# retab-dev/k-LLMs

Measured on NVIDIA H100. Metric: consensus records/sec at n=16 (1M x 32-field); achieved HBM GB/s vs peak, higher is better.
Workload: dtype i32 codes / f64 values

## Files before the change

### k_llms_b200/csrc/kc_jsongpu.cu

```cuda
#include <cuda_runtime.h>

#include <algorithm>
#include <atomic>
#include <chrono>
#include <cstdio>
#include <cstdlib>
#include <cstring>
#include <mutex>
#include <string>
#include <thread>
#include <vector>

#include <cub/device/device_scan.cuh>
#include <nvtx3/nvToolsExt.h>

#include "../../include/kllms_b200.h"
#include "kc_internal.h"
#include "kc_jsongpu.cuh"

namespace {

using kc::js::Chunk;
using kc::js::Tok;

struct DBuf {
    void *p = nullptr;
    size_t cap = 0;
    int reserve(size_t need) {
        if (p && need <= cap) return KC_OK;
        if (p) cudaFree(p);
        p = nullptr;
        cap = 0;
        need += need / 8 + 256;
        if (cudaMalloc(&p, need) != cudaSuccess) {
            cudaGetLastError();
            return kc_fail(KC_ENOMEM, "kc_consolidate_json_packed: cudaMalloc(%zu) failed", need);
        }
        cap = need;
        return KC_OK;
    }
    template <typename T>
    T *as() const { return static_cast<T *>(p); }
};

struct PBuf {
    void *p = nullptr;
    size_t cap = 0;
    int reserve(size_t need) {
        if (p && need <= cap) return KC_OK;
        if (p) cudaFreeHost(p);
        p = nullptr;
        cap = 0;
        need += need / 8 + 256;
        if (cudaHostAlloc(&p, need, cudaHostAllocDefault) != cudaSuccess) {
            cudaGetLastError();
            return kc_fail(KC_ENOMEM, "kc_consolidate_json_packed: cudaHostAlloc(%zu) failed", need);
        }
        cap = need;
        return KC_OK;
    }
    template <typename T>
    T *as() const { return static_cast<T *>(p); }
};

struct Worker {
    int device = -1;
    cudaStream_t stream = nullptr;
    cudaEvent_t ev[7] = {};
    DBuf text, off, fcount, slot, status, vbase, xbase, counters, toks, fdesc, piece_c, piece_l, vcells, xcells, win, vmeta, xvalue, xmeta,
        len_c, len_l, out_c, out_l, scan_tmp, mcount, scount, ccount, mchars, mstr_off, mgrp_off, midx, mavg, nest, gpos;
    PBuf h_small;
    PBuf h_scan;
    bool busy = false;
    int init(int dev) {
        if (device == dev) return KC_OK;
        KC_CUDA_I(cudaStreamCreateWithFlags(&stream, cudaStreamNonBlocking));
        for (auto &e : ev) KC_CUDA_I(cudaEventCreate(&e));
        device = dev;
        return KC_OK;
    }
};

std::mutex g_pool_mu;
std::vector<Worker *> g_workers;

Worker *acquire_worker(int device) {
    std::lock_guard<std::mutex> lock(g_pool_mu);
    for (Worker *w : g_workers)
        if (!w->busy && w->device == device) {
            w->busy = true;
            return w;
        }
    Worker *w = new Worker;
    w->busy = true;
    g_workers.push_back(w);
    return w;
}
void release_worker(Worker *w) {
    std::lock_guard<std::mutex> lock(g_pool_mu);
    w->busy = false;
}

struct PinnedBlob {
    char *p = nullptr;
    size_t cap = 0;
};
std::vector<PinnedBlob> g_blob_pool;

PinnedBlob acquire_blob(size_t need) {
    {
        std::lock_guard<std::mutex> lock(g_pool_mu);
        int best = -1;
        for (int i = 0; i < (int)g_blob_pool.size(); ++i)
            if (g_blob_pool[i].cap >= need && (best < 0 || g_blob_pool[i].cap < g_blob_pool[best].cap)) best = i;
        if (best >= 0) {
            PinnedBlob b = g_blob_pool[best];
            g_blob_pool.erase(g_blob_pool.begin() + best);
            return b;
        }
    }
    PinnedBlob b;
    void *p = nullptr;
    if (cudaHostAlloc(&p, need, cudaHostAllocDefault) != cudaSuccess) {
        cudaGetLastError();
        return b;
    }
    b.p = (char *)p;
    b.cap = need;
    return b;
}
void release_blob(PinnedBlob b) {
    if (!b.p) return;
    std::lock_guard<std::mutex> lock(g_pool_mu);
    size_t n_small = 0, n_large = 0;
    for (auto &x : g_blob_pool) (x.cap <= ((size_t)4 << 20) ? n_small : n_large)++;
    if (b.cap <= ((size_t)4 << 20) && n_small < 64) {
        g_blob_pool.push_back(b);
        return;
    }
    if (n_large >= 4 || b.cap <= ((size_t)4 << 20)) {
        int smallest = -1;
        for (int i = 0; i < (int)g_blob_pool.size(); ++i)
            if (g_blob_pool[i].cap > ((size_t)4 << 20) && (smallest < 0 || g_blob_pool[i].cap < g_blob_pool[smallest].cap)) smallest = i;
        if (smallest < 0 || g_blob_pool[smallest].cap >= b.cap) {
            cudaFreeHost(b.p);
            return;
        }
        cudaFreeHost(g_blob_pool[smallest].p);
        g_blob_pool.erase(g_blob_pool.begin() + smallest);
    }
    g_blob_pool.push_back(b);
}

int team_size(int n) {
    int t = 2;
    while (t < n && t < 32) t *= 2;
    return t;
}

}

struct kc_json_result {
    int64_t R = 0;
    PinnedBlob blob;
    std::atomic<int64_t> used{0};
    std::vector<int64_t> c_off, c_len, l_off, l_len;
    std::vector<uint8_t> status, why;
    std::string heap;
    kc_json_stats stats{};
};

namespace {

struct ChunkStage {
    float h2d = 0, plan = 0, kernels = 0, emit = 0, d2h = 0;
};

int run_chunk(Worker &w, const char *h_text, const int64_t *h_off, int64_t r0, int64_t r1, int32_t n, double rel_eps, double abs_eps,
              int sm_count, kc_json_result &res, ChunkStage &st) {
    const int64_t Rc = r1 - r0;
    const int64_t b0 = h_off[r0 * n], b1 = h_off[r1 * n];
    const size_t bytes = (size_t)(b1 - b0);
    if (bytes >= ((size_t)1 << 32)) return kc_fail(KC_EINVAL, "kc_consolidate_json_packed: chunk of %zu bytes", bytes);
    cudaStream_t s = w.stream;
    int rc;
#define R_(call)          \
    do {                  \
        rc = (call);      \
        if (rc) return rc; \
    } while (0)
    R_(w.text.reserve(bytes + 16));
    R_(w.off.reserve((size_t)(Rc * n + 1) * 8));
    R_(w.fcount.reserve((size_t)(Rc + 1) * 4));
    R_(w.slot.reserve((size_t)(Rc + 1) * 4));
    R_(w.status.reserve((size_t)Rc));
    R_(w.nest.reserve((size_t)Rc));
    R_(w.vbase.reserve((size_t)Rc * 4));
    R_(w.xbase.reserve((size_t)Rc * 4));
    R_(w.counters.reserve(32));
    R_(w.mcount.reserve((size_t)(Rc + 1) * 4));
    R_(w.scount.reserve((size_t)(Rc + 1) * 4));
    R_(w.ccount.reserve((size_t)(Rc + 1) * 4));
    R_(w.len_c.reserve((size_t)(Rc + 1) * 8));
    R_(w.len_l.reserve((size_t)(Rc + 1) * 8));
    R_(w.h_small.reserve(64));
    R_(w.h_scan.reserve((size_t)(Rc + 1) * 16 + (size_t)Rc));
    size_t tmp_bytes = 0, tmp_bytes32 = 0;
    cub::DeviceScan::ExclusiveSum(nullptr, tmp_bytes, (const int64_t *)nullptr, (int64_t *)nullptr, (int)(Rc + 1), s);
    cub::DeviceScan::ExclusiveSum(nullptr, tmp_bytes32, (const uint32_t *)nullptr, (uint32_t *)nullptr, (int)(Rc + 1), s);
    R_(w.scan_tmp.reserve(std::max(tmp_bytes, tmp_bytes32) + 256));

    Chunk ch{};
    ch.text = w.text.as<uint8_t>();
    ch.off = w.off.as<int64_t>();
    ch.R = (int32_t)Rc;
    ch.n = n;
    ch.fcount = w.fcount.as<uint32_t>();
    ch.slot = w.slot.as<uint32_t>();
    ch.status = w.status.as<uint8_t>();
    ch.nest = w.nest.as<uint8_t>();
    ch.vbase = w.vbase.as<uint32_t>();
    ch.xbase = w.xbase.as<uint32_t>();
    ch.counters = w.counters.as<unsigned long long>();
    ch.mcount = w.mcount.as<uint32_t>();
    ch.scount = w.scount.as<uint32_t>();
    ch.ccount = w.ccount.as<uint32_t>();
    ch.len_c = w.len_c.as<int64_t>();
    ch.len_l = w.len_l.as<int64_t>();

    nvtxRangePushA("kc_json: H2D texts");
    KC_CUDA_I(cudaEventRecord(w.ev[0], s));
    KC_CUDA_I(cudaMemcpyAsync(w.text.p, h_text + b0, bytes, cudaMemcpyHostToDevice, s));
    KC_CUDA_I(cudaMemcpyAsync(w.off.p, h_off + r0 * n, (size_t)(Rc * n + 1) * 8, cudaMemcpyHostToDevice, s));
    KC_CUDA_I(cudaEventRecord(w.ev[1], s));
    nvtxRangePop();
    nvtxRangePushA("kc_json: plan (A0 count, A1 scan/type/encode)");

    const int team = team_size(n);
    const int tpw = 32 / team;
    auto grid_for = [&](int64_t threads_needed) {
        const int64_t blocks = (threads_needed + 127) / 128;
        return (int)std::max<int64_t>(1, std::min<int64_t>(blocks, (int64_t)sm_count * 16));
    };
    KC_CUDA_I(cudaMemsetAsync(ch.fcount + Rc, 0, 4, s));
    kc::js::count_kernel<<<grid_for(Rc), 128, 0, s>>>(ch);
    KC_CUDA_I(cudaGetLastError());
    size_t tb = w.scan_tmp.cap;
    KC_CUDA_I(cub::DeviceScan::ExclusiveSum(w.scan_tmp.p, tb, (const uint32_t *)ch.fcount, ch.slot, (int)(Rc + 1), s));
    uint32_t *h_total = w.h_small.as<uint32_t>();
    KC_CUDA_I(cudaMemcpyAsync(h_total, ch.slot + Rc, 4, cudaMemcpyDeviceToHost, s));
    KC_CUDA_I(cudaStreamSynchronize(s));
    const size_t T = *h_total;
    const size_t Tn = T * (size_t)n;
    R_(w.toks.reserve(std::max<size_t>(Tn, 1) * sizeof(Tok)));
    R_(w.fdesc.reserve(std::max<size_t>(T, 1) * 4));
    R_(w.gpos.reserve(std::max<size_t>(T, 1) * 4));
    R_(w.piece_c.reserve(std::max<size_t>(T, 1) * 4));
    R_(w.piece_l.reserve(std::max<size_t>(T, 1) * 4));
    R_(w.vcells.reserve(std::max<size_t>(Tn, 16)));
    R_(w.xcells.reserve(std::max<size_t>(Tn, 2) * 8));
    R_(w.win.reserve(std::max<size_t>(T, 1) * 4));
    R_(w.vmeta.reserve(std::max<size_t>(T, 1) * 4));
    R_(w.xvalue.reserve(std::max<size_t>(T, 1) * 8));
    R_(w.xmeta.reserve(std::max<size_t>(T, 1) * 4));
    ch.toks = w.toks.as<Tok>();
    ch.fdesc = w.fdesc.as<uint32_t>();
    ch.gpos = w.gpos.as<uint32_t>();
    ch.piece_c = w.piece_c.as<uint32_t>();
    ch.piece_l = w.piece_l.as<uint32_t>();
    ch.vcells = w.vcells.as<int8_t>();
    ch.xcells = w.xcells.as<double>();
    ch.vmeta = w.vmeta.as<uint32_t>();
    ch.xvalue = w.xvalue.as<double>();
    ch.xmeta = w.xmeta.as<uint32_t>();
    KC_CUDA_I(cudaMemsetAsync(w.counters.p, 0, 24, s));
    KC_CUDA_I(cudaMemsetAsync(w.mcount.p, 0, (size_t)(Rc + 1) * 4, s));
    KC_CUDA_I(cudaMemsetAsync(w.scount.p, 0, (size_t)(Rc + 1) * 4, s));
    KC_CUDA_I(cudaMemsetAsync(w.ccount.p, 0, (size_t)(Rc + 1) * 4, s));
    KC_CUDA_I(cudaMemsetAsync(w.vcells.p, 0xFF, std::max<size_t>(Tn, 16), s));
    KC_CUDA_I(cudaMemsetAsync(w.xcells.p, 0, std::max<size_t>(Tn, 2) * 8, s));
    int64_t gv = 0, gx = 0, gm = 0;
    if (T) {
        const int64_t rounds = (Rc + tpw - 1) / tpw;
        kc::js::plan_kernel<<<grid_for(rounds * 32), 128, 0, s>>>(ch, team);
        KC_CUDA_I(cudaGetLastError());
        unsigned long long *h_cnt = w.h_small.as<unsigned long long>() + 1;
        KC_CUDA_I(cudaMemcpyAsync(h_cnt, w.counters.p, 24, cudaMemcpyDeviceToHost, s));
        KC_CUDA_I(cudaStreamSynchronize(s));
        gv = (int64_t)h_cnt[0];
        gx = (int64_t)h_cnt[1];
        gm = (int64_t)h_cnt[2];
    }
    if (gm) {
        R_(w.mchars.reserve(bytes + 16));
        R_(w.mstr_off.reserve((Tn + 2) * 4));
        R_(w.mgrp_off.reserve((T + 2) * 4));
        R_(w.midx.reserve((T + 1) * 4));
        R_(w.mavg.reserve((T + 1) * 8));
        ch.mchars = w.mchars.as<uint8_t>();
        ch.mstr_off = w.mstr_off.as<int32_t>();
        ch.mgrp_off = w.mgrp_off.as<int32_t>();
        ch.midx = w.midx.as<int32_t>();
        ch.mavg = w.mavg.as<double>();
        for (uint32_t *cnt : {ch.mcount, ch.scount, ch.ccount}) {
            tb = w.scan_tmp.cap;
            KC_CUDA_I(cub::DeviceScan::ExclusiveSum(w.scan_tmp.p, tb, (const uint32_t *)cnt, cnt, (int)(Rc + 1), s));
        }
        const int64_t rounds = (Rc + tpw - 1) / tpw;
        kc::js::medoid_kernel<<<grid_for(rounds * 32), 128, 0, s>>>(ch, team);
        KC_CUDA_I(cudaGetLastError());
    }
    KC_CUDA_I(cudaEventRecord(w.ev[2], s));
    nvtxRangePop();
    nvtxRangePushA("kc_json: K1 vote + K2 numeric + K4 medoid");
    if (gv) R_(kc_vote_i8(ch.vcells, gv, n, nullptr, 1, w.win.as<int32_t>(), w.vmeta.as<uint32_t>(), s));
    if (gx) R_(kc_numeric_f64(ch.xcells, gx, n, rel_eps, abs_eps, w.xvalue.as<double>(), w.xmeta.as<uint32_t>(), s));
    if (gm) R_(kc_medoid_str(ch.mchars, ch.mstr_off, ch.mgrp_off, gm, std::max(2, n), w.midx.as<int32_t>(), w.mavg.as<double>(), s));
    KC_CUDA_I(cudaEventRecord(w.ev[3], s));
    nvtxRangePop();
    nvtxRangePushA("kc_json: emit (C0 lengths, C1 write)");
    KC_CUDA_I(cudaMemsetAsync(ch.len_c + Rc, 0, 8, s));
    KC_CUDA_I(cudaMemsetAsync(ch.len_l + Rc, 0, 8, s));
    {
        const int64_t rounds = (Rc + tpw - 1) / tpw;
        kc::js::len_kernel<<<grid_for(rounds * 32), 128, 0, s>>>(ch, team);
        KC_CUDA_I(cudaGetLastError());
    }
    tb = w.scan_tmp.cap;
    KC_CUDA_I(cub::DeviceScan::ExclusiveSum(w.scan_tmp.p, tb, (const int64_t *)ch.len_c, ch.len_c, (int)(Rc + 1), s));
    tb = w.scan_tmp.cap;
    KC_CUDA_I(cub::DeviceScan::ExclusiveSum(w.scan_tmp.p, tb, (const int64_t *)ch.len_l, ch.len_l, (int)(Rc + 1), s));
    int64_t *h_scan_c = w.h_scan.as<int64_t>(), *h_scan_l = h_scan_c + (Rc + 1);
    uint8_t *h_status = (uint8_t *)(h_scan_l + (Rc + 1));
    KC_CUDA_I(cudaMemcpyAsync(h_scan_c, ch.len_c, (size_t)(Rc + 1) * 8, cudaMemcpyDeviceToHost, s));
    KC_CUDA_I(cudaMemcpyAsync(h_scan_l, ch.len_l, (size_t)(Rc + 1) * 8, cudaMemcpyDeviceToHost, s));
    KC_CUDA_I(cudaMemcpyAsync(h_status, ch.status, (size_t)Rc, cudaMemcpyDeviceToHost, s));
    KC_CUDA_I(cudaStreamSynchronize(s));
    const int64_t out_c_bytes = h_scan_c[Rc], out_l_bytes = h_scan_l[Rc];
    R_(w.out_c.reserve((size_t)std::max<int64_t>(out_c_bytes, 1)));
    R_(w.out_l.reserve((size_t)std::max<int64_t>(out_l_bytes, 1)));
    ch.out_c = w.out_c.as<uint8_t>();
    ch.out_l = w.out_l.as<uint8_t>();
    if (out_c_bytes) {
        const int64_t rounds = (Rc + tpw - 1) / tpw;
        kc::js::write_kernel<<<grid_for(rounds * 32), 128, 0, s>>>(ch, team);
        KC_CUDA_I(cudaGetLastError());
    }
    KC_CUDA_I(cudaEventRecord(w.ev[4], s));
    nvtxRangePop();
    nvtxRangePushA("kc_json: D2H texts");
    const int64_t need = out_c_bytes + out_l_bytes;
    const int64_t pos = res.used.fetch_add(need);
    if (pos + need > (int64_t)res.blob.cap) {
        res.used.fetch_sub(need);
        for (int64_t r = r0; r < r1; ++r) {
            res.status[(size_t)r] = 1;
            res.why[(size_t)r] = (uint8_t)kc::js::D_TOO_LONG;
        }
        return KC_OK;
    }
    if (out_c_bytes) KC_CUDA_I(cudaMemcpyAsync(res.blob.p + pos, ch.out_c, (size_t)out_c_bytes, cudaMemcpyDeviceToHost, s));
    if (out_l_bytes) KC_CUDA_I(cudaMemcpyAsync(res.blob.p + pos + out_c_bytes, ch.out_l, (size_t)out_l_bytes, cudaMemcpyDeviceToHost, s));
    KC_CUDA_I(cudaEventRecord(w.ev[5], s));
    KC_CUDA_I(cudaStreamSynchronize(s));
    nvtxRangePop();
    for (int64_t i = 0; i < Rc; ++i) {
        const int64_t r = r0 + i;
        res.status[(size_t)r] = h_status[i] ? 1 : 0;
        res.why[(size_t)r] = h_status[i];
        res.c_off[(size_t)r] = pos + h_scan_c[i];
        res.c_len[(size_t)r] = h_scan_c[i + 1] - h_scan_c[i];
        res.l_off[(size_t)r] = pos + out_c_bytes + h_scan_l[i];
        res.l_len[(size_t)r] = h_scan_l[i + 1] - h_scan_l[i];
    }
    float ms = 0;
    cudaEventElapsedTime(&ms, w.ev[0], w.ev[1]); st.h2d += ms;
    cudaEventElapsedTime(&ms, w.ev[1], w.ev[2]); st.plan += ms;
    cudaEventElapsedTime(&ms, w.ev[2], w.ev[3]); st.kernels += ms;
    cudaEventElapsedTime(&ms, w.ev[3], w.ev[4]); st.emit += ms;
    cudaEventElapsedTime(&ms, w.ev[4], w.ev[5]); st.d2h += ms;
#undef R_
    return KC_OK;
}

}

extern "C" {

int kc_consolidate_json_packed(const char *h_text, const int64_t *h_off, int64_t n_records, int32_t n, double rel_eps, double abs_eps,
                               int device, int32_t threads, uint32_t flags, kc_json_result **out) {
    if (!out) return kc_fail(KC_EINVAL, "kc_consolidate_json_packed: NULL out");
    *out = nullptr;
    if (n < 2 || n > KC_MAX_CANDIDATES) return kc_fail(KC_EINVAL, "kc_consolidate_json_packed: n=%d outside [2,%d]", n, KC_MAX_CANDIDATES);
    if (n_records < 0 || (n_records && (!h_text || !h_off))) return kc_fail(KC_EINVAL, "kc_consolidate_json_packed: bad arguments");
    if (!(rel_eps >= 0.0) || !(abs_eps >= 0.0)) return kc_fail(KC_EINVAL, "kc_consolidate_json_packed: rel_eps/abs_eps must be >= 0");
    const auto t_start = std::chrono::steady_clock::now();
    int prev = 0;
    KC_CUDA_I(cudaGetDevice(&prev));
    KC_CUDA_I(cudaSetDevice(device));
    int sm_count = 0, cc_major = 0;
    KC_CUDA_I(cudaDeviceGetAttribute(&sm_count, cudaDevAttrMultiProcessorCount, device));
    KC_CUDA_I(cudaDeviceGetAttribute(&cc_major, cudaDevAttrComputeCapabilityMajor, device));
    if (cc_major != 9) {
        cudaSetDevice(prev);
        return kc_fail(KC_ENODEV, "device %d has compute capability %d.x; this library is sm_90a only", device, cc_major);
    }
    kc_json_result *res = new (std::nothrow) kc_json_result;
    if (!res) return kc_fail(KC_ENOMEM, "kc_consolidate_json_packed: out of memory");
    const int64_t R = n_records;
    res->R = R;
    res->c_off.assign((size_t)R, 0);
    res->c_len.assign((size_t)R, 0);
    res->l_off.assign((size_t)R, 0);
    res->l_len.assign((size_t)R, 0);
    res->status.assign((size_t)R, 1);
    res->why.assign((size_t)R, 0);
    const int64_t total_bytes = R ? h_off[R * n] - h_off[0] : 0;
    res->blob = acquire_blob((size_t)(total_bytes / n * 3 + (1 << 20)));
    if (!res->blob.p) {
        delete res;
        cudaSetDevice(prev);
        return kc_fail(KC_ENOMEM, "kc_consolidate_json_packed: cannot allocate the pinned output blob");
    }
    size_t chunk_bytes = (size_t)64 << 20;
    if (const char *e = getenv("KC_JSON_CHUNK_MB")) chunk_bytes = (size_t)std::min(1024, std::max(1, atoi(e))) << 20;
    std::vector<int64_t> cuts{0};
    {
        int64_t r = 0;
        while (r < R) {
            const int64_t start = h_off[r * n];
            int64_t lo = r + 1, hi = R;
            while (lo < hi) {
                const int64_t mid = lo + (hi - lo + 1) / 2;
                if ((size_t)(h_off[mid * n] - start) <= chunk_bytes) lo = mid;
                else hi = mid - 1;
            }
            r = lo;
            cuts.push_back(r);
        }
    }
    const int n_chunks = (int)cuts.size() - 1;
    int n_workers = 3;
    if (const char *e = getenv("KC_JSON_STREAMS")) n_workers = std::max(1, std::min(8, atoi(e)));
    n_workers = std::max(1, std::min(n_workers, n_chunks));
    std::vector<Worker *> workers;
    for (int i = 0; i < n_workers; ++i) workers.push_back(acquire_worker(device));
    std::vector<int> rcs((size_t)n_workers, KC_OK);
    std::vector<std::string> errs((size_t)n_workers);
    std::vector<ChunkStage> stages((size_t)n_workers);
    std::atomic<int> next{0};
    auto body = [&](int wi) {
        cudaSetDevice(device);
        Worker &w = *workers[(size_t)wi];
        int rc = w.init(device);
        while (!rc) {
            const int k = next.fetch_add(1);
            if (k >= n_chunks) break;
            rc = run_chunk(w, h_text, h_off, cuts[(size_t)k], cuts[(size_t)k + 1], n, rel_eps, abs_eps, sm_count, *res, stages[(size_t)wi]);
        }
        if (rc) {
            cudaStreamSynchronize(w.stream);
            errs[(size_t)wi] = kc_last_error();
        }
        rcs[(size_t)wi] = rc;
    };
    if (n_workers == 1) {
        body(0);
    } else {
        std::vector<std::thread> pool;
        for (int i = 0; i < n_workers; ++i) pool.emplace_back(body, i);
        for (auto &t : pool) t.join();
    }
    for (Worker *w : workers) release_worker(w);
    int rc = KC_OK;
    for (int i = 0; i < n_workers && !rc; ++i)
        if (rcs[(size_t)i]) rc = kc_fail(rcs[(size_t)i], "%s", errs[(size_t)i].c_str());
    const auto t_gpu = std::chrono::steady_clock::now();
    int64_t n_declined = 0, n_host = 0;
    if (!rc) {
        std::vector<int64_t> idx;
        for (int64_t r = 0; r < R; ++r)
            if (res->status[(size_t)r]) idx.push_back(r);
        n_declined = (int64_t)idx.size();
        if (!idx.empty() && !(flags & KC_JSON_DEVICE_ONLY)) {
            const int64_t D = (int64_t)idx.size();
            std::vector<const char *> texts((size_t)(D * n));
            std::vector<int64_t> lens((size_t)(D * n));
            for (int64_t i = 0; i < D; ++i)
                for (int32_t c = 0; c < n; ++c) {
                    const int64_t k = idx[(size_t)i] * n + c;
                    texts[(size_t)(i * n + c)] = h_text + h_off[k];
                    lens[(size_t)(i * n + c)] = h_off[k + 1] - h_off[k];
                }
            std::vector<char *> oc((size_t)D, nullptr), ol((size_t)D, nullptr);
            std::vector<uint8_t> hs((size_t)D, 1);
            rc = kc_consolidate_json(texts.data(), lens.data(), D, n, rel_eps, abs_eps, device, threads, oc.data(), ol.data(), hs.data());
            if (!rc) {
                int64_t pos = res->used.load(), extra = 0;
                for (int64_t i = 0; i < D; ++i)
                    if (hs[(size_t)i] == 0) extra += (int64_t)(strlen(oc[(size_t)i]) + strlen(ol[(size_t)i]));
                char *base = res->blob.p;
                if (pos + extra > (int64_t)res->blob.cap) {
                    res->heap.resize((size_t)(pos + extra));
                    memcpy(&res->heap[0], res->blob.p, (size_t)pos);
                    release_blob(res->blob);
                    res->blob = PinnedBlob{};
                    base = &res->heap[0];
                }
                for (int64_t i = 0; i < D; ++i) {
                    if (hs[(size_t)i] != 0) continue;
                    const int64_t r = idx[(size_t)i];
                    const size_t lc = strlen(oc[(size_t)i]), ll = strlen(ol[(size_t)i]);
                    memcpy(base + pos, oc[(size_t)i], lc);
                    memcpy(base + pos + lc, ol[(size_t)i], ll);
                    res->c_off[(size_t)r] = pos;
                    res->l_off[(size_t)r] = pos + (int64_t)lc;
                    res->c_len[(size_t)r] = (int64_t)lc;
                    res->l_len[(size_t)r] = (int64_t)ll;
                    res->status[(size_t)r] = 2;
                    pos += (int64_t)(lc + ll);
                    ++n_host;
                }
                res->used.store(pos);
            }
            kc_free_strings(oc.data(), D);
            kc_free_strings(ol.data(), D);
        }
    }
    cudaSetDevice(prev);
    if (rc) {
        release_blob(res->blob);
        delete res;
        return rc;
    }
    const auto t_end = std::chrono::steady_clock::now();
    auto ms = [](auto a, auto b) { return std::chrono::duration<double, std::milli>(b - a).count(); };
    kc_json_stats &s = res->stats;
    s.n_records = R;
    s.n_device = R - n_declined;
    s.n_host = n_host;
    s.n_python = n_declined - n_host;
    s.input_bytes = total_bytes;
    s.output_bytes = res->used.load();
    s.chunks = n_chunks;
    s.streams = n_workers;
    for (auto &g : stages) {
        s.h2d_ms += g.h2d;
        s.plan_ms += g.plan;
        s.kernel_ms += g.kernels;
        s.emit_ms += g.emit;
        s.d2h_ms += g.d2h;
    }
    s.device_path_wall_ms = ms(t_start, t_gpu);
    s.host_path_wall_ms = ms(t_gpu, t_end);
    s.wall_ms = ms(t_start, t_end);
    *out = res;
    return KC_OK;
}

int kc_json_result_view(kc_json_result *res, const char **text, const int64_t **content_off, const int64_t **content_len,
                        const int64_t **likelihoods_off, const int64_t **likelihoods_len, const uint8_t **status, const uint8_t **why,
                        kc_json_stats *stats) {
    if (!res) return kc_fail(KC_EINVAL, "kc_json_result_view: NULL result");
    if (text) *text = res->blob.p ? res->blob.p : res->heap.data();
    if (content_off) *content_off = res->c_off.data();
    if (content_len) *content_len = res->c_len.data();
    if (likelihoods_off) *likelihoods_off = res->l_off.data();
    if (likelihoods_len) *likelihoods_len = res->l_len.data();
    if (status) *status = res->status.data();
    if (why) *why = res->why.data();
    if (stats) *stats = res->stats;
    return KC_OK;
}

void kc_json_result_free(kc_json_result *res) {
    if (!res) return;
    release_blob(res->blob);
    delete res;
}


struct kc_debug_jsongpu {
    std::vector<int64_t> off;
    std::vector<uint8_t> text;
    int32_t n = 0;
    int64_t R = 0;
    std::vector<uint32_t> fcount, slot, fdesc, gpos, vbase, xbase, piece_c, piece_l;
    std::vector<uint8_t> status, nest;
    std::vector<Tok> toks;
    unsigned long long counters[3] = {0, 0, 0};
    std::vector<uint32_t> mcount, scount, ccount;
    std::vector<uint8_t> mchars;
    std::vector<int32_t> mstr_off, mgrp_off;
    std::vector<int8_t> vcells;
    std::vector<double> xcells;
    std::vector<int64_t> len_c, len_l;
    std::vector<uint8_t> out_c, out_l;
    Chunk ch{};
};

int kc_debug_jsongpu_plan(const char *h_text, const int64_t *h_off, int64_t n_records, int32_t n, kc_debug_jsongpu **out) {
    if (!h_text || !h_off || !out || n < 2 || n > KC_MAX_CANDIDATES || n_records < 0) return KC_EINVAL;
    kc_debug_jsongpu *h = new kc_debug_jsongpu;
    const int64_t R = n_records;
    h->R = R;
    h->n = n;
    h->off.assign(h_off, h_off + R * n + 1);
    h->text.assign((const uint8_t *)h_text + h_off[0], (const uint8_t *)h_text + h_off[R * n]);
    h->fcount.assign((size_t)R + 1, 0);
    h->slot.assign((size_t)R + 1, 0);
    h->status.assign((size_t)R, 0);
    h->nest.assign((size_t)R, 0);
    h->vbase.assign((size_t)R, 0);
    h->xbase.assign((size_t)R, 0);
    h->len_c.assign((size_t)R + 1, 0);
    h->len_l.assign((size_t)R + 1, 0);
    h->mcount.assign((size_t)R + 1, 0);
    h->scount.assign((size_t)R + 1, 0);
    h->ccount.assign((size_t)R + 1, 0);
    Chunk &ch = h->ch;
    ch.text = h->text.data();
    ch.off = h->off.data();
    ch.R = (int32_t)R;
    ch.n = n;
    ch.fcount = h->fcount.data();
    ch.slot = h->slot.data();
    ch.status = h->status.data();
    ch.nest = h->nest.data();
    ch.vbase = h->vbase.data();
    ch.xbase = h->xbase.data();
    ch.counters = h->counters;
    ch.mcount = h->mcount.data();
    ch.scount = h->scount.data();
    ch.ccount = h->ccount.data();
    ch.len_c = h->len_c.data();
    ch.len_l = h->len_l.data();
    for (int32_t r = 0; r < R; ++r) kc::js::count_record(ch, r);
    for (int64_t r = 0; r < R; ++r) h->slot[(size_t)r + 1] = h->slot[(size_t)r] + h->fcount[(size_t)r];
    const size_t T = h->slot[(size_t)R];
    h->toks.assign(std::max<size_t>(T * n, 1), Tok{});
    h->fdesc.assign(std::max<size_t>(T, 1), 0);
    h->gpos.assign(std::max<size_t>(T, 1), 0);
    h->piece_c.assign(std::max<size_t>(T, 1), 0);
    h->piece_l.assign(std::max<size_t>(T, 1), 0);
    h->vcells.assign(std::max<size_t>(T * n, 16), (int8_t)-1);
    h->xcells.assign(std::max<size_t>(T * n, 2), 0.0);
    ch.toks = h->toks.data();
    ch.fdesc = h->fdesc.data();
    ch.gpos = h->gpos.data();
    ch.piece_c = h->piece_c.data();
    ch.piece_l = h->piece_l.data();
    ch.vcells = h->vcells.data();
    ch.xcells = h->xcells.data();
    const int team = team_size(n);
    for (int32_t r = 0; r < R; ++r) {
        for (int lane = 0; lane < team; ++lane) kc::js::parse_phase(ch, r, lane, team);
        for (int lane = 0; lane < team; ++lane) kc::js::type_phase(ch, r, lane, team);
        for (int lane = 0; lane < team; ++lane) kc::js::order_phase(ch, r, lane, team);
        kc::js::slots_phase(ch, r);
        for (int lane = 0; lane < team; ++lane) kc::js::encode_phase(ch, r, lane, team);
    }
    for (std::vector<uint32_t> *cnt : {&h->mcount, &h->scount, &h->ccount}) {
        uint32_t acc = 0;
        for (auto &x : *cnt) {
            const uint32_t v = x;
            x = acc;
            acc += v;
        }
    }
    h->mchars.assign((size_t)h->ccount[(size_t)R] + 1, 0);
    h->mstr_off.assign((size_t)h->scount[(size_t)R] + 1, 0);
    h->mgrp_off.assign((size_t)h->mcount[(size_t)R] + 1, 0);
    ch.mchars = h->mchars.data();
    ch.mstr_off = h->mstr_off.data();
    ch.mgrp_off = h->mgrp_off.data();
    for (int32_t r = 0; r < R; ++r)
        for (int lane = 0; lane < team; ++lane) kc::js::medoid_phase(ch, r, lane, team);
    *out = h;
    return KC_OK;
}

int kc_debug_jsongpu_medoid_inputs(const kc_debug_jsongpu *h, const uint8_t **chars, const int32_t **str_off, const int32_t **grp_off,
                                   int64_t *n_groups) {
    if (!h) return KC_EINVAL;
    if (chars) *chars = h->mchars.data();
    if (str_off) *str_off = h->mstr_off.data();
    if (grp_off) *grp_off = h->mgrp_off.data();
    if (n_groups) *n_groups = (int64_t)h->counters[2];
    return KC_OK;
}

int kc_debug_jsongpu_set_medoid(kc_debug_jsongpu *h, const int32_t *medoid_idx, const double *medoid_avg) {
    if (!h) return KC_EINVAL;
    h->ch.midx = medoid_idx;
    h->ch.mavg = medoid_avg;
    return KC_OK;
}

int kc_debug_jsongpu_inputs(const kc_debug_jsongpu *h, const int8_t **vote_cells, int64_t *n_vote_groups, const double **num_cells,
                            int64_t *n_num_groups, const uint8_t **status) {
    if (!h) return KC_EINVAL;
    if (vote_cells) *vote_cells = h->vcells.data();
    if (n_vote_groups) *n_vote_groups = (int64_t)h->counters[0];
    if (num_cells) *num_cells = h->xcells.data();
    if (n_num_groups) *n_num_groups = (int64_t)h->counters[1];
    if (status) *status = h->status.data();
    return KC_OK;
}

int kc_debug_jsongpu_emit(kc_debug_jsongpu *h, const uint32_t *vote_meta, const double *num_value, const uint32_t *num_meta,
                          const char **content, const int64_t **content_off, const char **likelihoods, const int64_t **likelihoods_off) {
    if (!h) return KC_EINVAL;
    Chunk &ch = h->ch;
    ch.vmeta = vote_meta;
    ch.xvalue = num_value;
    ch.xmeta = num_meta;
    const int64_t R = h->R;
    const int team = team_size(h->n);
    for (int32_t r = 0; r < R; ++r) {
        for (int lane = 0; lane < team; ++lane) kc::js::len_phase(ch, r, lane, team);
        kc::js::offsets_phase(ch, r);
    }
    int64_t ac = 0, al = 0;
// ... 165 lines not shown
```

Measured before the change: 1.004 billion.

## Prefetch chunk inputs on a dedicated copy stream through a slot ring

Host-to-device copies of chunk text and offsets move out of each worker's stream onto a dedicated copy thread and stream. That thread fills a ring of device slots ahead of the workers, with events and a condition-variable pipe enforcing fill/free ordering. This lets H2D transfers overlap kernel work on other chunks. Result allocation now runs concurrently with the first copies, and offsets are staged through pinned host buffers. The cost is extra threads, extra device memory for the slots, and more complex synchronisation.

```diff
diff --git a/k_llms_b200/csrc/kc_jsongpu.cu b/k_llms_b200/csrc/kc_jsongpu.cu
--- a/k_llms_b200/csrc/kc_jsongpu.cu
+++ b/k_llms_b200/csrc/kc_jsongpu.cu
@@ -3,6 +3,7 @@
 #include <algorithm>
 #include <atomic>
 #include <chrono>
+#include <condition_variable>
 #include <cstdio>
 #include <cstdlib>
 #include <cstring>
@@ -67,7 +68,7 @@
     int device = -1;
     cudaStream_t stream = nullptr;
     cudaEvent_t ev[7] = {};
-    DBuf text, off, fcount, slot, status, vbase, xbase, counters, toks, fdesc, piece_c, piece_l, vcells, xcells, win, vmeta, xvalue, xmeta,
+    DBuf fcount, slot, status, vbase, xbase, counters, toks, fdesc, piece_c, piece_l, vcells, xcells, win, vmeta, xvalue, xmeta,
         len_c, len_l, out_c, out_l, scan_tmp, mcount, scount, ccount, mchars, mstr_off, mgrp_off, midx, mavg, nest, gpos;
     PBuf h_small;
     PBuf h_scan;
@@ -101,6 +102,112 @@
     w->busy = false;
 }
 
+struct Slot {
+    DBuf text, off;
+    PBuf h_off;
+    cudaEvent_t start = nullptr;
+    cudaEvent_t filled = nullptr;
+    cudaEvent_t freed = nullptr;
+    bool timed = true;
+};
+
+struct Ring {
+    int device = -1;
+    cudaStream_t copy = nullptr;
+    std::vector<Slot *> slots;
+    bool busy = false;
+    int init(int dev, int n_slots) {
+        if (device != dev) {
+            KC_CUDA_I(cudaStreamCreateWithFlags(&copy, cudaStreamNonBlocking));
+            device = dev;
+        }
+        while ((int)slots.size() < n_slots) {
+            Slot *sl = new Slot;
+            KC_CUDA_I(cudaEventCreate(&sl->start));
+            KC_CUDA_I(cudaEventCreate(&sl->filled));
+            KC_CUDA_I(cudaEventCreateWithFlags(&sl->freed, cudaEventDisableTiming));
+            slots.push_back(sl);
+        }
+        return KC_OK;
+    }
+};
+
+std::vector<Ring *> g_rings;
+
+Ring *acquire_ring(int device) {
+    std::lock_guard<std::mutex> lock(g_pool_mu);
+    for (Ring *g : g_rings)
+        if (!g->busy && g->device == device) {
+            g->busy = true;
+            return g;
+        }
+    Ring *g = new Ring;
+    g->busy = true;
+    g_rings.push_back(g);
+    return g;
+}
+void release_ring(Ring *g) {
+    std::lock_guard<std::mutex> lock(g_pool_mu);
+    g->busy = false;
+}
+
+struct Pipe {
+    std::mutex mu;
+    std::condition_variable cv;
+    int64_t filled = 0;
+    std::vector<uint8_t> freed;
+    bool abort = false;
+    explicit Pipe(int n_chunks) : freed((size_t)n_chunks, 0) {}
+    void publish_filled(int64_t k) {
+        { std::lock_guard<std::mutex> lock(mu); filled = k + 1; }
+        cv.notify_all();
+    }
+    void publish_freed(int64_t k) {
+        { std::lock_guard<std::mutex> lock(mu); freed[(size_t)k] = 1; }
+        cv.notify_all();
+    }
+    void stop() {
+        { std::lock_guard<std::mutex> lock(mu); abort = true; }
+        cv.notify_all();
+    }
+    bool wait_filled(int64_t k) {
+        std::unique_lock<std::mutex> lock(mu);
+        cv.wait(lock, [&] { return abort || filled > k; });
+        return filled > k;
+    }
+    bool wait_freed(int64_t k) {
+        std::unique_lock<std::mutex> lock(mu);
+        cv.wait(lock, [&] { return abort || freed[(size_t)k]; });
+        return freed[(size_t)k] != 0;
+    }
+};
+
+void account_fill(Slot &sl, double *h2d_ms) {
+    if (sl.timed) return;
+    float ms = 0;
+    cudaEventSynchronize(sl.filled);
+    if (cudaEventElapsedTime(&ms, sl.start, sl.filled) == cudaSuccess) *h2d_ms += ms;
+    cudaGetLastError();
+    sl.timed = true;
+}
+
+int fill_slot(Slot &sl, const char *h_text, const int64_t *h_off, int64_t r0, int64_t r1, int32_t n, cudaStream_t s, double *h2d_ms) {
+    const int64_t b0 = h_off[r0 * n], b1 = h_off[r1 * n];
+    const size_t bytes = (size_t)(b1 - b0), off_bytes = (size_t)((r1 - r0) * n + 1) * 8;
+    if (bytes >= ((size_t)1 << 32)) return kc_fail(KC_EINVAL, "kc_consolidate_json_packed: chunk of %zu bytes", bytes);
+    account_fill(sl, h2d_ms);
+    if (bytes + 16 > sl.text.cap || off_bytes > sl.off.cap) cudaEventSynchronize(sl.freed);
+    int rc;
+    if ((rc = sl.text.reserve(bytes + 16)) || (rc = sl.off.reserve(off_bytes)) || (rc = sl.h_off.reserve(off_bytes))) return rc;
+    memcpy(sl.h_off.p, h_off + r0 * n, off_bytes);
+    KC_CUDA_I(cudaEventRecord(sl.start, s));
+    KC_CUDA_I(cudaMemcpyAsync(sl.text.p, h_text + b0, bytes, cudaMemcpyHostToDevice, s));
+    KC_CUDA_I(cudaMemcpyAsync(sl.off.p, sl.h_off.p, off_bytes, cudaMemcpyHostToDevice, s));
+    KC_CUDA_I(cudaEventRecord(sl.filled, s));
+    sl.timed = false;
+    return KC_OK;
+}
+
 struct PinnedBlob {
     char *p = nullptr;
     size_t cap = 0;
@@ -173,15 +280,15 @@
 namespace {
 
 struct ChunkStage {
-    float h2d = 0, plan = 0, kernels = 0, emit = 0, d2h = 0;
+    float plan = 0, kernels = 0, emit = 0, d2h = 0;
 };
 
-int run_chunk(Worker &w, const char *h_text, const int64_t *h_off, int64_t r0, int64_t r1, int32_t n, double rel_eps, double abs_eps,
-              int sm_count, kc_json_result &res, ChunkStage &st) {
+template <typename OnFreed>
+int run_chunk(Worker &w, Slot &sl, const int64_t *h_off, int64_t r0, int64_t r1, int32_t n, double rel_eps, double abs_eps,
+              int sm_count, kc_json_result &res, ChunkStage &st, OnFreed on_freed) {
     const int64_t Rc = r1 - r0;
     const int64_t b0 = h_off[r0 * n], b1 = h_off[r1 * n];
     const size_t bytes = (size_t)(b1 - b0);
-    if (bytes >= ((size_t)1 << 32)) return kc_fail(KC_EINVAL, "kc_consolidate_json_packed: chunk of %zu bytes", bytes);
     cudaStream_t s = w.stream;
     int rc;
 #define R_(call)          \
@@ -189,8 +296,6 @@
         rc = (call);      \
         if (rc) return rc; \
     } while (0)
-    R_(w.text.reserve(bytes + 16));
-    R_(w.off.reserve((size_t)(Rc * n + 1) * 8));
     R_(w.fcount.reserve((size_t)(Rc + 1) * 4));
     R_(w.slot.reserve((size_t)(Rc + 1) * 4));
     R_(w.status.reserve((size_t)Rc));
@@ -211,8 +316,8 @@
     R_(w.scan_tmp.reserve(std::max(tmp_bytes, tmp_bytes32) + 256));
 
     Chunk ch{};
-    ch.text = w.text.as<uint8_t>();
-    ch.off = w.off.as<int64_t>();
+    ch.text = sl.text.as<uint8_t>();
+    ch.off = sl.off.as<int64_t>();
     ch.R = (int32_t)Rc;
     ch.n = n;
     ch.fcount = w.fcount.as<uint32_t>();
@@ -228,12 +333,8 @@
     ch.len_c = w.len_c.as<int64_t>();
     ch.len_l = w.len_l.as<int64_t>();
 
-    nvtxRangePushA("kc_json: H2D texts");
-    KC_CUDA_I(cudaEventRecord(w.ev[0], s));
-    KC_CUDA_I(cudaMemcpyAsync(w.text.p, h_text + b0, bytes, cudaMemcpyHostToDevice, s));
-    KC_CUDA_I(cudaMemcpyAsync(w.off.p, h_off + r0 * n, (size_t)(Rc * n + 1) * 8, cudaMemcpyHostToDevice, s));
+    KC_CUDA_I(cudaStreamWaitEvent(s, sl.filled, 0));
     KC_CUDA_I(cudaEventRecord(w.ev[1], s));
-    nvtxRangePop();
     nvtxRangePushA("kc_json: plan (A0 count, A1 scan/type/encode)");
 
     const int team = team_size(n);
@@ -346,6 +447,8 @@
         kc::js::write_kernel<<<grid_for(rounds * 32), 128, 0, s>>>(ch, team);
         KC_CUDA_I(cudaGetLastError());
     }
+    KC_CUDA_I(cudaEventRecord(sl.freed, s));
+    on_freed();
     KC_CUDA_I(cudaEventRecord(w.ev[4], s));
     nvtxRangePop();
     nvtxRangePushA("kc_json: D2H texts");
@@ -374,7 +477,6 @@
         res.l_len[(size_t)r] = h_scan_l[i + 1] - h_scan_l[i];
     }
     float ms = 0;
-    cudaEventElapsedTime(&ms, w.ev[0], w.ev[1]); st.h2d += ms;
     cudaEventElapsedTime(&ms, w.ev[1], w.ev[2]); st.plan += ms;
     cudaEventElapsedTime(&ms, w.ev[2], w.ev[3]); st.kernels += ms;
     cudaEventElapsedTime(&ms, w.ev[3], w.ev[4]); st.emit += ms;
@@ -405,23 +507,8 @@
         cudaSetDevice(prev);
         return kc_fail(KC_ENODEV, "device %d has compute capability %d.x; this library is sm_90a only", device, cc_major);
     }
-    kc_json_result *res = new (std::nothrow) kc_json_result;
-    if (!res) return kc_fail(KC_ENOMEM, "kc_consolidate_json_packed: out of memory");
     const int64_t R = n_records;
-    res->R = R;
-    res->c_off.assign((size_t)R, 0);
-    res->c_len.assign((size_t)R, 0);
-    res->l_off.assign((size_t)R, 0);
-    res->l_len.assign((size_t)R, 0);
-    res->status.assign((size_t)R, 1);
-    res->why.assign((size_t)R, 0);
     const int64_t total_bytes = R ? h_off[R * n] - h_off[0] : 0;
-    res->blob = acquire_blob((size_t)(total_bytes / n * 3 + (1 << 20)));
-    if (!res->blob.p) {
-        delete res;
-        cudaSetDevice(prev);
-        return kc_fail(KC_ENOMEM, "kc_consolidate_json_packed: cannot allocate the pinned output blob");
-    }
     size_t chunk_bytes = (size_t)64 << 20;
     if (const char *e = getenv("KC_JSON_CHUNK_MB")) chunk_bytes = (size_t)std::min(1024, std::max(1, atoi(e))) << 20;
     std::vector<int64_t> cuts{0};
@@ -445,35 +532,89 @@
     n_workers = std::max(1, std::min(n_workers, n_chunks));
     std::vector<Worker *> workers;
     for (int i = 0; i < n_workers; ++i) workers.push_back(acquire_worker(device));
-    std::vector<int> rcs((size_t)n_workers, KC_OK);
-    std::vector<std::string> errs((size_t)n_workers);
+    const int n_slots = std::max(1, std::min(n_chunks, n_workers + 4));
+    Ring *ring = acquire_ring(device);
+    std::vector<int> rcs((size_t)n_workers + 1, KC_OK);
+    std::vector<std::string> errs((size_t)n_workers + 1);
     std::vector<ChunkStage> stages((size_t)n_workers);
+    double h2d_ms = 0;
+    Pipe pipe(n_chunks);
     std::atomic<int> next{0};
+    kc_json_result *res = nullptr;
     auto body = [&](int wi) {
         cudaSetDevice(device);
         Worker &w = *workers[(size_t)wi];
         int rc = w.init(device);
         while (!rc) {
             const int k = next.fetch_add(1);
-            if (k >= n_chunks) break;
-            rc = run_chunk(w, h_text, h_off, cuts[(size_t)k], cuts[(size_t)k + 1], n, rel_eps, abs_eps, sm_count, *res, stages[(size_t)wi]);
+            if (k >= n_chunks || !pipe.wait_filled(k)) break;
+            rc = run_chunk(w, *ring->slots[(size_t)(k % n_slots)], h_off, cuts[(size_t)k], cuts[(size_t)k + 1], n, rel_eps, abs_eps, sm_count,
+                           *res, stages[(size_t)wi], [&] { pipe.publish_freed(k); });
         }
         if (rc) {
+            pipe.stop();
             cudaStreamSynchronize(w.stream);
             errs[(size_t)wi] = kc_last_error();
         }
         rcs[(size_t)wi] = rc;
     };
-    if (n_workers == 1) {
-        body(0);
-    } else {
+    auto copy_chunks = [&](cudaStream_t s) -> int {
+        for (int k = 0; k < n_chunks; ++k) {
+            Slot &sl = *ring->slots[(size_t)(k % n_slots)];
+            if (k >= n_slots) {
+                if (!pipe.wait_freed(k - n_slots)) return KC_OK;
+                KC_CUDA_I(cudaStreamWaitEvent(s, sl.freed, 0));
+            }
+            const int rc = fill_slot(sl, h_text, h_off, cuts[(size_t)k], cuts[(size_t)k + 1], n, s, &h2d_ms);
+            if (rc) return rc;
+            pipe.publish_filled(k);
+        }
+        return KC_OK;
+    };
+    auto copier = [&](cudaStream_t s) {
+        cudaSetDevice(device);
+        const int rc = copy_chunks(s);
+        if (rc) {
+            pipe.stop();
+            cudaStreamSynchronize(s);
+            errs[(size_t)n_workers] = kc_last_error();
+        }
+        rcs[(size_t)n_workers] = rc;
+    };
+    int rc = ring->init(device, n_slots);
+    std::thread copy_thread;
+    if (!rc && n_chunks > 1) copy_thread = std::thread(copier, ring->copy);
+    if (!rc) {
+        res = new (std::nothrow) kc_json_result;
+        if (res) {
+            res->R = R;
+            res->c_off.assign((size_t)R, 0);
+            res->c_len.assign((size_t)R, 0);
+            res->l_off.assign((size_t)R, 0);
+            res->l_len.assign((size_t)R, 0);
+            res->status.assign((size_t)R, 1);
+            res->why.assign((size_t)R, 0);
+            res->blob = acquire_blob((size_t)(total_bytes / n * 3 + (1 << 20)));
+        }
+        if (!res) rc = kc_fail(KC_ENOMEM, "kc_consolidate_json_packed: out of memory");
+        else if (!res->blob.p) rc = kc_fail(KC_ENOMEM, "kc_consolidate_json_packed: cannot allocate the pinned output blob");
+        if (rc) pipe.stop();
+    }
+    if (!rc && n_chunks <= 1) {
+        rc = workers[0]->init(device);
+        if (!rc) copier(workers[0]->stream);
+        if (!rc && !rcs[(size_t)n_workers]) body(0);
+    } else if (!rc) {
         std::vector<std::thread> pool;
         for (int i = 0; i < n_workers; ++i) pool.emplace_back(body, i);
         for (auto &t : pool) t.join();
     }
+    if (copy_thread.joinable()) copy_thread.join();
+    cudaStreamSynchronize(ring->copy);
+    for (int i = 0; i < n_slots && i < (int)ring->slots.size(); ++i) account_fill(*ring->slots[(size_t)i], &h2d_ms);
+    release_ring(ring);
     for (Worker *w : workers) release_worker(w);
-    int rc = KC_OK;
-    for (int i = 0; i < n_workers && !rc; ++i)
+    for (int i = 0; i <= n_workers && !rc; ++i)
         if (rcs[(size_t)i]) rc = kc_fail(rcs[(size_t)i], "%s", errs[(size_t)i].c_str());
     const auto t_gpu = std::chrono::steady_clock::now();
     int64_t n_declined = 0, n_host = 0;
@@ -529,7 +670,7 @@
     }
     cudaSetDevice(prev);
     if (rc) {
-        release_blob(res->blob);
+        if (res) release_blob(res->blob);
         delete res;
         return rc;
     }
@@ -544,8 +685,8 @@
     s.output_bytes = res->used.load();
     s.chunks = n_chunks;
     s.streams = n_workers;
+    s.h2d_ms = h2d_ms;
     for (auto &g : stages) {
-        s.h2d_ms += g.h2d;
         s.plan_ms += g.plan;
         s.kernel_ms += g.kernels;
         s.emit_ms += g.emit;
```

Result: no change. 1.003 billion (median of 6 runs) (-0.1%).

## Prefetch chunk texts through a shared H2D copy-stream ring buffer

Applied to the files above, without the earlier changes.

Moves host-to-device copies of chunk texts and offsets out of each worker's stream onto a dedicated copy stream. A ring of n_workers+2 device slots is filled ahead by the main thread and coordinated with events and a condition variable, so transfers for later chunks overlap with kernels on earlier ones. It also replaces zero-initialized result vectors with uninitialized arrays, avoiding a fill pass over per-record outputs. The cost is more threading and event complexity, pageable offset staging through pinned buffers, and extra device memory for the slots.

```diff
diff --git a/k_llms_b200/csrc/kc_jsongpu.cu b/k_llms_b200/csrc/kc_jsongpu.cu
--- a/k_llms_b200/csrc/kc_jsongpu.cu
+++ b/k_llms_b200/csrc/kc_jsongpu.cu
@@ -5,7 +5,9 @@
 #include <chrono>
 #include <cstdio>
 #include <cstdlib>
+#include <condition_variable>
 #include <cstring>
+#include <memory>
 #include <mutex>
 #include <string>
 #include <thread>
@@ -66,8 +68,8 @@
 struct Worker {
     int device = -1;
     cudaStream_t stream = nullptr;
-    cudaEvent_t ev[7] = {};
-    DBuf text, off, fcount, slot, status, vbase, xbase, counters, toks, fdesc, piece_c, piece_l, vcells, xcells, win, vmeta, xvalue, xmeta,
+    cudaEvent_t ev[5] = {};
+    DBuf fcount, slot, status, vbase, xbase, counters, toks, fdesc, piece_c, piece_l, vcells, xcells, win, vmeta, xvalue, xmeta,
         len_c, len_l, out_c, out_l, scan_tmp, mcount, scount, ccount, mchars, mstr_off, mgrp_off, midx, mavg, nest, gpos;
     PBuf h_small;
     PBuf h_scan;
@@ -152,6 +154,135 @@
     g_blob_pool.push_back(b);
 }
 
+struct TextRing {
+    static constexpr int kMaxSlots = 8 + 2;
+    struct Slot {
+        DBuf text, off;
+        PBuf h_off;
+        cudaEvent_t filled = nullptr, released = nullptr;
+        cudaEvent_t t0 = nullptr, t1 = nullptr;
+        int64_t filled_seq = -1, released_seq = -1;
+        bool timed = false;
+    };
+    int device = -1;
+    cudaStream_t copy = nullptr;
+    Slot slots[kMaxSlots];
+    int B = 0;
+    std::mutex mu;
+    std::condition_variable cv;
+    bool abort = false;
+    bool busy = false;
+    float h2d_ms = 0;
+
+    int init(int dev) {
+        if (device == dev) return KC_OK;
+        KC_CUDA_I(cudaStreamCreateWithFlags(&copy, cudaStreamNonBlocking));
+        for (Slot &sl : slots) {
+            KC_CUDA_I(cudaEventCreateWithFlags(&sl.filled, cudaEventDisableTiming));
+            KC_CUDA_I(cudaEventCreateWithFlags(&sl.released, cudaEventDisableTiming));
+            KC_CUDA_I(cudaEventCreate(&sl.t0));
+            KC_CUDA_I(cudaEventCreate(&sl.t1));
+        }
+        device = dev;
+        return KC_OK;
+    }
+    void begin(int n_slots) {
+        B = n_slots;
+        abort = false;
+        h2d_ms = 0;
+        for (Slot &sl : slots) {
+            sl.filled_seq = sl.released_seq = -1;
+            sl.timed = false;
+        }
+    }
+    void stop() {
+        {
+            std::lock_guard<std::mutex> lock(mu);
+            abort = true;
+        }
+        cv.notify_all();
+    }
+    int add_time(Slot &sl) {
+        if (!sl.timed) return KC_OK;
+        float ms = 0;
+        KC_CUDA_I(cudaEventSynchronize(sl.t1));
+        KC_CUDA_I(cudaEventElapsedTime(&ms, sl.t0, sl.t1));
+        h2d_ms += ms;
+        sl.timed = false;
+        return KC_OK;
+    }
+
+    int fill(int64_t k, const char *h_text, const int64_t *h_off, bool off_pinned, int64_t r0, int64_t r1, int32_t n) {
+        Slot &sl = slots[k % B];
+        {
+            std::unique_lock<std::mutex> lock(mu);
+            cv.wait(lock, [&] { return abort || sl.released_seq >= k - B; });
+            if (abort) return KC_OK;
+        }
+        const int64_t b0 = h_off[r0 * n];
+        const size_t bytes = (size_t)(h_off[r1 * n] - b0), off_bytes = (size_t)((r1 - r0) * n + 1) * 8;
+        if (bytes >= ((size_t)1 << 32)) return kc_fail(KC_EINVAL, "kc_consolidate_json_packed: chunk of %zu bytes", bytes);
+        if (bytes + 16 > sl.text.cap || off_bytes > sl.off.cap) KC_CUDA_I(cudaEventSynchronize(sl.released));
+        int rc;
+        if ((rc = sl.text.reserve(bytes + 16)) || (rc = sl.off.reserve(off_bytes))) return rc;
+        KC_CUDA_I(cudaStreamWaitEvent(copy, sl.released, 0));
+        if ((rc = add_time(sl))) return rc;
+        KC_CUDA_I(cudaEventRecord(sl.t0, copy));
+        KC_CUDA_I(cudaMemcpyAsync(sl.text.p, h_text + b0, bytes, cudaMemcpyHostToDevice, copy));
+        const int64_t *src = h_off + r0 * n;
+        if (!off_pinned) {
+            KC_CUDA_I(cudaEventSynchronize(sl.filled));
+            if ((rc = sl.h_off.reserve(off_bytes))) return rc;
+            memcpy(sl.h_off.p, src, off_bytes);
+            src = sl.h_off.as<int64_t>();
+        }
+        KC_CUDA_I(cudaMemcpyAsync(sl.off.p, src, off_bytes, cudaMemcpyHostToDevice, copy));
+        KC_CUDA_I(cudaEventRecord(sl.t1, copy));
+        KC_CUDA_I(cudaEventRecord(sl.filled, copy));
+        sl.timed = true;
+        {
+            std::lock_guard<std::mutex> lock(mu);
+            sl.filled_seq = k;
+        }
+        cv.notify_all();
+        return KC_OK;
+    }
+    bool wait_filled(int64_t k) {
+        std::unique_lock<std::mutex> lock(mu);
+        cv.wait(lock, [&] { return abort || slots[k % B].filled_seq >= k; });
+        return !abort;
+    }
+    void release(int64_t k, cudaStream_t s) {
+        Slot &sl = slots[k % B];
+        const bool recorded = cudaEventRecord(sl.released, s) == cudaSuccess;
+        {
+            std::lock_guard<std::mutex> lock(mu);
+            if (recorded) sl.released_seq = k;
+            else abort = true;
+        }
+        cv.notify_all();
+    }
+};
+
+std::vector<TextRing *> g_rings;
+
+TextRing *acquire_ring(int device) {
+    std::lock_guard<std::mutex> lock(g_pool_mu);
+    for (TextRing *r : g_rings)
+        if (!r->busy && r->device == device) {
+            r->busy = true;
+            return r;
+        }
+    TextRing *r = new TextRing;
+    r->busy = true;
+    g_rings.push_back(r);
+    return r;
+}
+void release_ring(TextRing *r) {
+    std::lock_guard<std::mutex> lock(g_pool_mu);
+    r->busy = false;
+}
+
 int team_size(int n) {
     int t = 2;
     while (t < n && t < 32) t *= 2;
@@ -164,8 +295,8 @@
     int64_t R = 0;
     PinnedBlob blob;
     std::atomic<int64_t> used{0};
-    std::vector<int64_t> c_off, c_len, l_off, l_len;
-    std::vector<uint8_t> status, why;
+    std::unique_ptr<int64_t[]> c_off, c_len, l_off, l_len;
+    std::unique_ptr<uint8_t[]> status, why;
     std::string heap;
     kc_json_stats stats{};
 };
@@ -173,24 +304,34 @@
 namespace {
 
 struct ChunkStage {
-    float h2d = 0, plan = 0, kernels = 0, emit = 0, d2h = 0;
+    float plan = 0, kernels = 0, emit = 0, d2h = 0;
 };
 
-int run_chunk(Worker &w, const char *h_text, const int64_t *h_off, int64_t r0, int64_t r1, int32_t n, double rel_eps, double abs_eps,
-              int sm_count, kc_json_result &res, ChunkStage &st) {
+struct SlotRelease {
+    TextRing &ring;
+    int64_t k;
+    cudaStream_t s;
+    bool done = false;
+    void operator()() {
+        if (!done) ring.release(k, s);
+        done = true;
+    }
+    ~SlotRelease() { (*this)(); }
+};
+
+int run_chunk(Worker &w, TextRing &ring, int64_t k, const int64_t *h_off, int64_t r0, int64_t r1, int32_t n, double rel_eps,
+              double abs_eps, int sm_count, kc_json_result &res, ChunkStage &st) {
     const int64_t Rc = r1 - r0;
-    const int64_t b0 = h_off[r0 * n], b1 = h_off[r1 * n];
-    const size_t bytes = (size_t)(b1 - b0);
-    if (bytes >= ((size_t)1 << 32)) return kc_fail(KC_EINVAL, "kc_consolidate_json_packed: chunk of %zu bytes", bytes);
+    const size_t bytes = (size_t)(h_off[r1 * n] - h_off[r0 * n]);
     cudaStream_t s = w.stream;
+    TextRing::Slot &sl = ring.slots[k % ring.B];
+    SlotRelease release{ring, k, s};
     int rc;
 #define R_(call)          \
     do {                  \
         rc = (call);      \
         if (rc) return rc; \
     } while (0)
-    R_(w.text.reserve(bytes + 16));
-    R_(w.off.reserve((size_t)(Rc * n + 1) * 8));
     R_(w.fcount.reserve((size_t)(Rc + 1) * 4));
     R_(w.slot.reserve((size_t)(Rc + 1) * 4));
     R_(w.status.reserve((size_t)Rc));
@@ -211,8 +352,8 @@
     R_(w.scan_tmp.reserve(std::max(tmp_bytes, tmp_bytes32) + 256));
 
     Chunk ch{};
-    ch.text = w.text.as<uint8_t>();
-    ch.off = w.off.as<int64_t>();
+    ch.text = sl.text.as<uint8_t>();
+    ch.off = sl.off.as<int64_t>();
     ch.R = (int32_t)Rc;
     ch.n = n;
     ch.fcount = w.fcount.as<uint32_t>();
@@ -228,12 +369,8 @@
     ch.len_c = w.len_c.as<int64_t>();
     ch.len_l = w.len_l.as<int64_t>();
 
-    nvtxRangePushA("kc_json: H2D texts");
+    KC_CUDA_I(cudaStreamWaitEvent(s, sl.filled, 0));
     KC_CUDA_I(cudaEventRecord(w.ev[0], s));
-    KC_CUDA_I(cudaMemcpyAsync(w.text.p, h_text + b0, bytes, cudaMemcpyHostToDevice, s));
-    KC_CUDA_I(cudaMemcpyAsync(w.off.p, h_off + r0 * n, (size_t)(Rc * n + 1) * 8, cudaMemcpyHostToDevice, s));
-    KC_CUDA_I(cudaEventRecord(w.ev[1], s));
-    nvtxRangePop();
     nvtxRangePushA("kc_json: plan (A0 count, A1 scan/type/encode)");
 
     const int team = team_size(n);
@@ -310,13 +447,13 @@
         kc::js::medoid_kernel<<<grid_for(rounds * 32), 128, 0, s>>>(ch, team);
         KC_CUDA_I(cudaGetLastError());
     }
-    KC_CUDA_I(cudaEventRecord(w.ev[2], s));
+    KC_CUDA_I(cudaEventRecord(w.ev[1], s));
     nvtxRangePop();
     nvtxRangePushA("kc_json: K1 vote + K2 numeric + K4 medoid");
     if (gv) R_(kc_vote_i8(ch.vcells, gv, n, nullptr, 1, w.win.as<int32_t>(), w.vmeta.as<uint32_t>(), s));
     if (gx) R_(kc_numeric_f64(ch.xcells, gx, n, rel_eps, abs_eps, w.xvalue.as<double>(), w.xmeta.as<uint32_t>(), s));
     if (gm) R_(kc_medoid_str(ch.mchars, ch.mstr_off, ch.mgrp_off, gm, std::max(2, n), w.midx.as<int32_t>(), w.mavg.as<double>(), s));
-    KC_CUDA_I(cudaEventRecord(w.ev[3], s));
+    KC_CUDA_I(cudaEventRecord(w.ev[2], s));
     nvtxRangePop();
     nvtxRangePushA("kc_json: emit (C0 lengths, C1 write)");
     KC_CUDA_I(cudaMemsetAsync(ch.len_c + Rc, 0, 8, s));
@@ -346,7 +483,8 @@
         kc::js::write_kernel<<<grid_for(rounds * 32), 128, 0, s>>>(ch, team);
         KC_CUDA_I(cudaGetLastError());
     }
-    KC_CUDA_I(cudaEventRecord(w.ev[4], s));
+    release();
+    KC_CUDA_I(cudaEventRecord(w.ev[3], s));
     nvtxRangePop();
     nvtxRangePushA("kc_json: D2H texts");
     const int64_t need = out_c_bytes + out_l_bytes;
@@ -356,12 +494,13 @@
         for (int64_t r = r0; r < r1; ++r) {
             res.status[(size_t)r] = 1;
             res.why[(size_t)r] = (uint8_t)kc::js::D_TOO_LONG;
+            res.c_off[(size_t)r] = res.c_len[(size_t)r] = res.l_off[(size_t)r] = res.l_len[(size_t)r] = 0;
         }
         return KC_OK;
     }
     if (out_c_bytes) KC_CUDA_I(cudaMemcpyAsync(res.blob.p + pos, ch.out_c, (size_t)out_c_bytes, cudaMemcpyDeviceToHost, s));
     if (out_l_bytes) KC_CUDA_I(cudaMemcpyAsync(res.blob.p + pos + out_c_bytes, ch.out_l, (size_t)out_l_bytes, cudaMemcpyDeviceToHost, s));
-    KC_CUDA_I(cudaEventRecord(w.ev[5], s));
+    KC_CUDA_I(cudaEventRecord(w.ev[4], s));
     KC_CUDA_I(cudaStreamSynchronize(s));
     nvtxRangePop();
     for (int64_t i = 0; i < Rc; ++i) {
@@ -374,11 +513,10 @@
         res.l_len[(size_t)r] = h_scan_l[i + 1] - h_scan_l[i];
     }
     float ms = 0;
-    cudaEventElapsedTime(&ms, w.ev[0], w.ev[1]); st.h2d += ms;
-    cudaEventElapsedTime(&ms, w.ev[1], w.ev[2]); st.plan += ms;
-    cudaEventElapsedTime(&ms, w.ev[2], w.ev[3]); st.kernels += ms;
-    cudaEventElapsedTime(&ms, w.ev[3], w.ev[4]); st.emit += ms;
-    cudaEventElapsedTime(&ms, w.ev[4], w.ev[5]); st.d2h += ms;
+    cudaEventElapsedTime(&ms, w.ev[0], w.ev[1]); st.plan += ms;
+    cudaEventElapsedTime(&ms, w.ev[1], w.ev[2]); st.kernels += ms;
+    cudaEventElapsedTime(&ms, w.ev[2], w.ev[3]); st.emit += ms;
+    cudaEventElapsedTime(&ms, w.ev[3], w.ev[4]); st.d2h += ms;
 #undef R_
     return KC_OK;
 }
@@ -409,12 +547,14 @@
     if (!res) return kc_fail(KC_ENOMEM, "kc_consolidate_json_packed: out of memory");
     const int64_t R = n_records;
     res->R = R;
-    res->c_off.assign((size_t)R, 0);
-    res->c_len.assign((size_t)R, 0);
-    res->l_off.assign((size_t)R, 0);
-    res->l_len.assign((size_t)R, 0);
-    res->status.assign((size_t)R, 1);
-    res->why.assign((size_t)R, 0);
+    for (auto *a : {&res->c_off, &res->c_len, &res->l_off, &res->l_len}) a->reset(new (std::nothrow) int64_t[(size_t)R]);
+    res->status.reset(new (std::nothrow) uint8_t[(size_t)R]);
+    res->why.reset(new (std::nothrow) uint8_t[(size_t)R]);
+    if (!res->c_off || !res->c_len || !res->l_off || !res->l_len || !res->status || !res->why) {
+        delete res;
+        cudaSetDevice(prev);
+        return kc_fail(KC_ENOMEM, "kc_consolidate_json_packed: out of memory");
+    }
     const int64_t total_bytes = R ? h_off[R * n] - h_off[0] : 0;
     res->blob = acquire_blob((size_t)(total_bytes / n * 3 + (1 << 20)));
     if (!res->blob.p) {
@@ -445,36 +585,53 @@
     n_workers = std::max(1, std::min(n_workers, n_chunks));
     std::vector<Worker *> workers;
     for (int i = 0; i < n_workers; ++i) workers.push_back(acquire_worker(device));
+    TextRing *ring = acquire_ring(device);
+    int rc = ring->init(device);
     std::vector<int> rcs((size_t)n_workers, KC_OK);
     std::vector<std::string> errs((size_t)n_workers);
     std::vector<ChunkStage> stages((size_t)n_workers);
-    std::atomic<int> next{0};
-    auto body = [&](int wi) {
-        cudaSetDevice(device);
-        Worker &w = *workers[(size_t)wi];
-        int rc = w.init(device);
-        while (!rc) {
-            const int k = next.fetch_add(1);
-            if (k >= n_chunks) break;
-            rc = run_chunk(w, h_text, h_off, cuts[(size_t)k], cuts[(size_t)k + 1], n, rel_eps, abs_eps, sm_count, *res, stages[(size_t)wi]);
-        }
-        if (rc) {
-            cudaStreamSynchronize(w.stream);
-            errs[(size_t)wi] = kc_last_error();
-        }
-        rcs[(size_t)wi] = rc;
-    };
-    if (n_workers == 1) {
-        body(0);
-    } else {
+    if (!rc) {
+        ring->begin(n_workers + 2);
+        cudaPointerAttributes pa{};
+        const bool off_pinned = R && cudaPointerGetAttributes(&pa, h_off) == cudaSuccess && pa.type == cudaMemoryTypeHost;
+        cudaGetLastError();
+        std::atomic<int> next{0};
+        auto body = [&](int wi) {
+            cudaSetDevice(device);
+            Worker &w = *workers[(size_t)wi];
+            int wrc = w.init(device);
+            while (!wrc) {
+                const int k = next.fetch_add(1);
+                if (k >= n_chunks || !ring->wait_filled(k)) break;
+                wrc = run_chunk(w, *ring, k, h_off, cuts[(size_t)k], cuts[(size_t)k + 1], n, rel_eps, abs_eps, sm_count, *res,
+                                stages[(size_t)wi]);
+            }
+            if (wrc) {
+                ring->stop();
+                cudaStreamSynchronize(w.stream);
+                errs[(size_t)wi] = kc_last_error();
+            }
+            rcs[(size_t)wi] = wrc;
+        };
         std::vector<std::thread> pool;
         for (int i = 0; i < n_workers; ++i) pool.emplace_back(body, i);
+        for (int k = 0; k < n_chunks && !rc; ++k) rc = ring->fill(k, h_text, h_off, off_pinned, cuts[(size_t)k], cuts[(size_t)k + 1], n);
+        std::string issue_err;
+        if (rc) {
+            issue_err = kc_last_error();
+            ring->stop();
+        }
         for (auto &t : pool) t.join();
-    }
+        cudaStreamSynchronize(ring->copy);
+        for (auto &sl : ring->slots)
+            if (!rc) rc = ring->add_time(sl);
+        if (rc && !issue_err.empty()) rc = kc_fail(rc, "%s", issue_err.c_str());
+        for (int i = 0; i < n_workers && !rc; ++i)
+            if (rcs[(size_t)i]) rc = kc_fail(rcs[(size_t)i], "%s", errs[(size_t)i].c_str());
+    }
+    const float h2d_ms = ring->h2d_ms;
+    release_ring(ring);
     for (Worker *w : workers) release_worker(w);
-    int rc = KC_OK;
-    for (int i = 0; i < n_workers && !rc; ++i)
-        if (rcs[(size_t)i]) rc = kc_fail(rcs[(size_t)i], "%s", errs[(size_t)i].c_str());
     const auto t_gpu = std::chrono::steady_clock::now();
     int64_t n_declined = 0, n_host = 0;
     if (!rc) {
@@ -544,8 +701,8 @@
     s.output_bytes = res->used.load();
     s.chunks = n_chunks;
     s.streams = n_workers;
+    s.h2d_ms = h2d_ms;
     for (auto &g : stages) {
-        s.h2d_ms += g.h2d;
         s.plan_ms += g.plan;
         s.kernel_ms += g.kernels;
         s.emit_ms += g.emit;
@@ -563,12 +720,12 @@
                         kc_json_stats *stats) {
     if (!res) return kc_fail(KC_EINVAL, "kc_json_result_view: NULL result");
     if (text) *text = res->blob.p ? res->blob.p : res->heap.data();
-    if (content_off) *content_off = res->c_off.data();
-    if (content_len) *content_len = res->c_len.data();
-    if (likelihoods_off) *likelihoods_off = res->l_off.data();
-    if (likelihoods_len) *likelihoods_len = res->l_len.data();
-    if (status) *status = res->status.data();
-    if (why) *why = res->why.data();
+    if (content_off) *content_off = res->c_off.get();
+    if (content_len) *content_len = res->c_len.get();
+    if (likelihoods_off) *likelihoods_off = res->l_off.get();
+    if (likelihoods_len) *likelihoods_len = res->l_len.get();
+    if (status) *status = res->status.get();
+    if (why) *why = res->why.get();
     if (stats) *stats = res->stats;
     return KC_OK;
 }
```

Measured after the change: 1.005 billion before, 1.006 billion after, median of 6. About the same (+0.1%).
